# whaiproject/BetaZero

Measured on AMD Instinct MI355X. Metric: selfplay_games_per_s, higher is better.
Workload: dtype bf16

## Files before the change

betazero_amd/csrc/bz_mcts.hip:

```cpp
#include <new>

#include <time.h>

#include "bz_common.h"
#include "bz_math.h"
#include "bz_rules.h"
#include "bz_fpu.h"
#include "bz_solver.h"
#include "bz_early_stop.h"
#include "bz_options.h"
#include "bz_pace.h"
#include "bz_gumbel_interior.h"
#include "bz_surprise.h"
#include "bz_value.h"
#include "bz_ownership.h"
#include "bz_resign.h"

using namespace bz;

namespace {

struct __attribute__((aligned(16))) Node { u64 own, opp, legal; u32 edge0, info; };
struct __attribute__((aligned(16))) Edge { u32 w0; float W; float P; u32 w3; };
static_assert(sizeof(Node) == 32 && sizeof(Edge) == 16, "layout");
// ... 2231 lines not shown
    const int tm = E.g_to_move[g];
    uint8_t* st = R.streak + i * 2 + (tm == 1 ? 0 : 1);
    int s;
    const bool fire = resign_step(q, R.threshold, R.consecutive, (int)*st, &s);
    *st = (uint8_t)s;
    if (!fire) return;
    if (R.side[i] == 0) { R.side[i] = (int8_t)tm; R.move[i] = E.g_moves[g]; R.q[i] = q; }
    if (out) return;
    const int nex = E.g_nex[g] < E.t_max ? E.g_nex[g] : E.t_max, w = -tm;
    const size_t rowbase = i * E.t_max;
    for (int t = 0; t < nex; ++t) E.ex_z[rowbase + t] = (int8_t)(w * E.ex_mover[rowbase + t]);
    E.ex_len[i] = nex;
    E.ex_winner[i] = (int8_t)w;
    atomicAdd(&E.flags[FLAG_FINISHED], 1u);
    E.g_state[g] = kStateResigned;
}
template <class G>
__global__ void __launch_bounds__(256) k_resign_finish(EngineDev E, int restart) {
    const int g = blockIdx.x * blockDim.x + threadIdx.x;
    if (g >= E.B || E.g_state[g] != kStateResigned) return;
    const int round = E.g_round[g];
    if (restart && round + 1 < E.rounds) { dev_start_game<G>(E, g, round + 1); return; }
    E.g_state[g] = 1;
}

__global__ void __launch_bounds__(256) k_pack_own(EngineDev E, OwnDev O, u64* fown, u64* fopp, int64_t cap) {
    dev_pack_walk(E, cap, [=](int i, size_t s, size_t d) {
        u64 a, b;
        ownership_row(O.fin_x[i], O.fin_o[i], (int)E.ex_mover[s], &a, &b);
        fown[d] = a; fopp[d] = b;
    });
}

struct __attribute__((aligned(64))) StoreHdr { u64 own, opp, epoch; u32 n_nodes, n_edges, ready, pad[7]; };
static_assert(sizeof(StoreHdr) == 64, "layout");
struct StoreDev {
    int S, D, n_idx, base;
    u32* n_used;
    u32* idx;
    StoreHdr* hdr;
    u32* mark;
    Node* nodes; Edge* edges; float* node_v; u64* tt;
};
constexpr int kCntSeededEvals = 11, kCntSeededSearches = 12, kCntStoreSaves = 13;
constexpr int kCntReplaySeeds = 14, kCntReplaySims = 15;

__device__ __forceinline__ u32 store_home(const StoreDev& St, u64 own, u64 opp) { return (u32)(hash_pos(own, opp) >> 20) & (u32)(St.n_idx - 1); }
__device__ __forceinline__ int store_find(const StoreDev& St, u64 own, u64 opp, u64 epoch, u32* at) {
    u32 p = store_home(St, own, opp);
    for (int k = 0; k < St.n_idx; ++k, p = (p + 1u) & (u32)(St.n_idx - 1)) {
        const u32 w = St.idx[p];
        if (w == 0u || w > (u32)St.S) { *at = p; return -1; }
        const StoreHdr& h = St.hdr[w - 1u];
        if (h.own == own && h.opp == opp && h.epoch == epoch) { *at = p; return (int)(w - 1u); }
    }
    *at = ~0u;
    return -1;
}
__device__ __forceinline__ bool store_depth_ok(const EngineDev& E, const StoreDev& St, int g) {
    const int d = E.g_moves[g] - St.base;
    return E.g_state[g] == 0 && d >= 0 && d < St.D;
}
__device__ __forceinline__ u32 tt_gen_before(u32 gen) { return gen == 1u ? kTtGenMax - 1u : gen - 1u; }

__device__ __forceinline__ bool tt_replay_from_prev(const EngineDev& E, int g, u32 i, u32 gen, u32 prev_nodes) {
    const Node nd = E.nodes[(size_t)g * E.ncap + i];
    if (nd.info & kTerm) return false;
#ifdef BZ_EXP_TT_WEAK_HASH
    const u64 h = hash_pos(nd.own, nd.opp) & 1u;
#else
    const u64 h = hash_pos(nd.own, nd.opp);
#endif
    const u32 tag = (u32)(h >> 32), gen_prev = tt_gen_before(gen);
    const u64* bucket = E.tt + ((size_t)g * (size_t)E.tt_buckets + (size_t)(h & (u64)(E.tt_buckets - 1))) * 16;
    u32 hit = ~0u;
    for (int s = 0; s < 16; ++s) {
        const u64 e = bucket[s];
        const u32 meta = (u32)(e >> 32), egen = meta >> kChildBits;
        const bool cur = egen == gen && (meta & kChildMask) < i, prv = prev_nodes != 0u && egen == gen_prev;
        if ((cur || prv) && (u32)e == tag) {
            const u32 key = ((prv ? 1u : 0u) << 20) | ((u32)s << 16) | (meta & kChildMask);
            hit = key < hit ? key : hit;
        }
    }
    if (hit == ~0u || (hit >> 20) == 0u) return false;
    const u32 x = hit & kChildMask;
    if (x == 0u || x >= prev_nodes) return false;
    const Node xn = E.nodes_alt[(size_t)g * E.ncap + x];
    return xn.own == nd.own && xn.opp == nd.opp && !(xn.info & kTerm) && (xn.info & 0xFFu) != 0u;
}

__global__ void __launch_bounds__(256) k_store_save(EngineDev E, StoreDev St, u32 gen, u64 epoch, const u32* budget) {
    __shared__ int claim[256];
    __shared__ u32 part[256];
    const int t = threadIdx.x;
    if ((int)blockIdx.x < E.B) {
        const int g = blockIdx.x;
        const GameHot& hot = E.hot[g];
        if (E.g_state[g] != 0 || hot.tt_gen != gen || hot.last_gen != gen || hot.prev_nodes == 0u || St.mark[g] != tt_gen_before(gen)) return;
        const u32 n = hot.n_nodes < (u32)E.ncap ? hot.n_nodes : (u32)E.ncap;
        u32 mine = 0;
        for (u32 i = 1u + (u32)t; i < n; i += 256u) mine += tt_replay_from_prev(E, g, i, gen, hot.prev_nodes) ? 1u : 0u;
        part[t] = mine;
        __syncthreads();
        for (int o = 128; o > 0; o >>= 1) { if (t < o) part[t] += part[t + o]; __syncthreads(); }
        if (t == 0 && part[0]) atomicAdd(reinterpret_cast<unsigned long long*>(E.counters) + kCntSeededEvals, (unsigned long long)part[0]);
        return;
    }
    const size_t ttn = (size_t)E.tt_buckets * 16;
    for (int g0 = 0; g0 < E.B; g0 += 256) {
        const int g = g0 + t;
        int c = -1;
        if (g < E.B && store_depth_ok(E, St, g) && E.hot[g].last_gen == gen && E.hot[g].tt_gen == gen && E.hot[g].n_nodes > 1u &&
            E.hot[g].n_nodes <= (u32)E.ncap && E.hot[g].n_edges <= (u32)E.ecap && !(budget && budget[g] < (u32)E.sims)) {
            const Node r = E.nodes[(size_t)g * E.ncap];
            u32 at;
            if (store_find(St, r.own, r.opp, epoch, &at) < 0) c = -2;
        }
        claim[t] = c;
        __syncthreads();
        if (t == 0) {
            for (int j = 0; j < 256; ++j) {
                if (claim[j] != -2) continue;
                claim[j] = -1;
                const u32 used = *St.n_used;
                if (used >= (u32)St.S) continue;
                const int gj = g0 + j;
                const Node r = E.nodes[(size_t)gj * E.ncap];
                u32 at;
                if (store_find(St, r.own, r.opp, epoch, &at) >= 0 || at == ~0u) continue;
                StoreHdr h{};
                h.own = r.own; h.opp = r.opp; h.epoch = epoch; h.n_nodes = E.hot[gj].n_nodes; h.n_edges = E.hot[gj].n_edges; h.ready = 0u;
                St.hdr[used] = h;
                St.idx[at] = used + 1u;
                *St.n_used = used + 1u;
                __threadfence();
                claim[j] = (int)used;
            }
        }
        __syncthreads();
        for (int j = 0; j < 256; ++j) {
            const int en = claim[j];
            if (en < 0) continue;
            const int gj = g0 + j;
            const u32 nn = St.hdr[en].n_nodes, ne = St.hdr[en].n_edges;
            const uint4* sn = reinterpret_cast<const uint4*>(E.nodes + (size_t)gj * E.ncap);
            uint4* dn = reinterpret_cast<uint4*>(St.nodes + (size_t)en * E.ncap);
            for (u32 k = t; k < nn * 2u; k += 256u) dn[k] = sn[k];
            const uint4* se = reinterpret_cast<const uint4*>(E.edges + (size_t)gj * E.ecap);
            uint4* de = reinterpret_cast<uint4*>(St.edges + (size_t)en * E.ecap);
            for (u32 k = t; k < ne; k += 256u) de[k] = se[k];
            const float* sv = E.node_v + (size_t)gj * E.ncap;
            float* dv = St.node_v + (size_t)en * E.ncap;
            for (u32 k = t; k < nn; k += 256u) dv[k] = sv[k];
            const u64* st = E.tt + (size_t)gj * ttn;
            u64* dt = St.tt + (size_t)en * ttn;
            for (size_t k = t; k < ttn; k += 256) {
                const u64 e = st[k];
                dt[k] = ((u32)(e >> 32) >> kChildBits) == gen ? e : 0ULL;
            }
        }
        __syncthreads();
        if (t == 0)
            for (int j = 0; j < 256; ++j)
                if (claim[j] >= 0) {
                    St.hdr[claim[j]].ready = 1u;
                    atomicAdd(reinterpret_cast<unsigned long long*>(E.counters) + kCntStoreSaves, 1ULL);
                }
        __syncthreads();
    }
}

__global__ void __launch_bounds__(256) k_store_seed(EngineDev E, StoreDev St, u32 gen, u64 epoch) {
    __shared__ int found;
    const int g = blockIdx.x, t = threadIdx.x;
    if (t == 0) {
        int en = -1;
        if (store_depth_ok(E, St, g)) {
            u32 at;
            en = store_find(St, E.g_own[g], E.g_opp[g], epoch, &at);
            if (en >= 0 && (St.hdr[en].ready == 0u || St.hdr[en].n_nodes > (u32)E.ncap || St.hdr[en].n_edges > (u32)E.ecap)) en = -1;
        }
        found = en;
    }
    __syncthreads();
    const int en = found;
    if (en < 0) return;
    const u32 nn = St.hdr[en].n_nodes, ne = St.hdr[en].n_edges;
    const uint4* sn = reinterpret_cast<const uint4*>(St.nodes + (size_t)en * E.ncap);
    uint4* dn = reinterpret_cast<uint4*>(E.nodes + (size_t)g * E.ncap);
    for (u32 k = t; k < nn * 2u; k += 256u) dn[k] = sn[k];
    const uint4* se = reinterpret_cast<const uint4*>(St.edges + (size_t)en * E.ecap);
    uint4* de = reinterpret_cast<uint4*>(E.edges + (size_t)g * E.ecap);
    for (u32 k = t; k < ne; k += 256u) de[k] = se[k];
    const float* sv = St.node_v + (size_t)en * E.ncap;
    float* dv = E.node_v + (size_t)g * E.ncap;
    for (u32 k = t; k < nn; k += 256u) dv[k] = sv[k];
    const size_t ttn = (size_t)E.tt_buckets * 16;
    const u64* st = St.tt + (size_t)en * ttn;
    u64* dt = E.tt + (size_t)g * ttn;
    for (size_t k = t; k < ttn; k += 256) {
        const u64 e = st[k];
// ... 643 lines not shown
}

static bool root_prep(const bz_engine* e) { return e->dev.dir_eps > 0.0f || e->gumbel.m > 0; }
static bool search_is_fused(const bz_engine* e) {
    const int ek = e->cfg.eval_kind;
    return (ek == BZ_EVAL_UNIFORM || ek == BZ_EVAL_HASH) && !e->dev.reuse && !root_prep(e) && engine_mode(e) == 0u;
}

constexpr int kPaceAutoSlots = 1024;
static int32_t paced_search(bz_engine* e, void* stream) {
    const int from_prev = e->seed_src;
    const bool plain = engine_mode(e) == 0u && !(e->dev.dir_eps > 0.0f) && !e->dev.reuse && !e->sym_on && e->dev.ecache == 2 &&
                       net_eval(e->cfg.eval_kind) && e->cfg.game != BZ_GAME_TTT && e->dev.compact;
    if (!plain || e->replay_seed == 0 || (e->replay_seed == 2 && e->dev.B <= kPaceAutoSlots)) return BZ_OK;
    const size_t lds = (size_t)e->dev.ncap * 8;
    const u32* mark = e->store.S > 0 ? e->store.mark : nullptr;
#define BZ_SEED(G) hipLaunchKernelGGL(k_replay_seed<G>, dim3(e->dev.B), dim3(G::GW), lds, (hipStream_t)stream, e->dev, e->search_seq, from_prev, mark)
    switch (e->cfg.game) {
    case BZ_GAME_REVERSI6: BZ_SEED(Reversi6); break;
    case BZ_GAME_REVERSI4: BZ_SEED(Reversi4); break;
    default: BZ_SEED(Reversi); break;
    }
#undef BZ_SEED
    BZ_LAUNCH_CHECK("k_replay_seed");
    e->paced = 1;
    return BZ_OK;
}

static int32_t store_save(bz_engine* e, void* stream) {
    if (e->store.S == 0) return BZ_OK;
    hipLaunchKernelGGL(k_store_save, dim3(e->dev.B + 1), dim3(256), 0, (hipStream_t)stream, e->dev, e->store, e->search_seq, e->eval_epoch,
                       cap_budgets(e));
    BZ_LAUNCH_CHECK("k_store_save");
    return BZ_OK;
}

BZ_EXPORT int32_t bz_engine_search(bz_engine* e, void* stream) {
    BZ_REQUIRE(e, "null engine");
    int ek = e->cfg.eval_kind;
    const bool noise = root_prep(e);
    if (search_is_fused(e)) {
        ProfScope ps(BZ_PROF_SEARCH_FUSED, stream);
        if (e->cfg.game == BZ_GAME_TTT && e->cfg.sims <= kTttFusedMaxSims && e->ttt_gw > 0) {
            const dim3 grid = grid_groups(e->dev.B, e->ttt_gw);
#define BZ_TTT_FUSED(GWN)                                                                                              \
    do {                                                                                                                \
        if (ek == BZ_EVAL_UNIFORM) hipLaunchKernelGGL((k_search_fused_ttt<GWN, true>), grid, dim3(256), 0, (hipStream_t)stream, e->dev); \
        else hipLaunchKernelGGL((k_search_fused_ttt<GWN, false>), grid, dim3(256), 0, (hipStream_t)stream, e->dev);     \
    } while (0)
            switch (e->ttt_gw) {
            case 1: BZ_TTT_FUSED(1); break;
            case 2: BZ_TTT_FUSED(2); break;
            case 8: BZ_TTT_FUSED(8); break;
            default: BZ_TTT_FUSED(4); break;
            }
#undef BZ_TTT_FUSED
            BZ_LAUNCH_CHECK("k_search_fused_ttt");
            return BZ_OK;
        }
        BZ_DISPATCH_G(e, k_search_fused, stream, e->dev, ek);
        return BZ_OK;
    }
    BZ_REQUIRE(ek != BZ_EVAL_EXTERNAL, "bz_engine_search: BZ_EVAL_EXTERNAL callers drive the step API");
    int32_t rc;
    if ((rc = bz_engine_root_begin(e, stream)) != BZ_OK) return rc;
    if ((rc = paced_search(e, stream)) != BZ_OK) return rc;
// ... 880 lines not shown
```

betazero_amd/csrc/bz_net.hip:

```cpp
#include <limits.h>
#include <math.h>
#include <stdlib.h>
#include <new>
#include <atomic>
#include <vector>

#include "bz_common.h"
#include "bz_math.h"
#include "bz_sym.h"
#include "bz_tower.h"

using namespace bz;

using namespace bz_tower;

struct bz_net {
    int C, NB, VH, max_batch;
    float *stem_w, *stem_b;
    float *conv_w, *conv_b;
    __bf16* conv_wf;
    __bf16 *stem_wf, *head_wf;
    __bf16 *conv_wf16, *stem_wf16;
    uint8_t *conv_wf8, *head_wf8;
    float *dq8, *head_dq8, *ones;
// ... 40 lines not shown
            int src[8];
#pragma unroll
            for (int j = 0; j < 8; ++j) {
                int cell = c0 + j, yy = (cell >> 3) + dy, xx = (cell & 7) + dx;
                src[j] = (yy < 0 || yy > 7 || xx < 0 || xx > 7) ? -1 : (yy * 8 + xx) * C;
            }
            const float* wt = w + (size_t)t * C * C + co;
            for (int ci = 0; ci < C; ++ci) {
                float wv = wt[(size_t)ci * C];
#pragma unroll
                for (int j = 0; j < 8; ++j)
                    if (src[j] >= 0) acc[j] = __builtin_fmaf(xs[src[j] + ci], wv, acc[j]);
            }
        }
#pragma unroll
        for (int j = 0; j < 8; ++j) {
            size_t o = ((size_t)pos * 64 + c0 + j) * C + co;
            float v = acc[j];
            if (skip) v = v + skip[o];
            out[o] = relu_f32(v);
        }
    }
}

typedef Tw<64, 2> TwS64;
typedef Tw<128, 1> TwS128;
typedef Tw<256, 1> TwS256;
typedef Tw<128, 4, true> TwM16;
typedef Tw<128, 4, true, 1> TwEdge;
constexpr int kSmallBatch = 256;
constexpr int kAdaptT1 = 256;
enum { kShapeLatency = 0, kShapeMiddle = 1, kShapeThroughput = 2, kShapes = 4 };

struct TowerArgs {
    const u64 *own, *opp;
    const u32* n_dev;
    int n, n_layers, VH;
    int lo, hi;
    u32* tally;
    const uint4* wf;
    const uint4 *wf16, *stem_wf16;
    const float* bias;
    const uint4* stem_wf;
    const float* stem_b;
    const uint4* head_wf;
    const uint4 *wf8, *head_wf8;
    const float *dq8, *head_dq8, *ones;
    const float *pol_b, *val_b;
    const float *polfc_wT, *polfc_b;
    const float *v1_wT, *v1_b, *v2_w, *v2_b;
    float *logits, *value;
};

__device__ __forceinline__ unsigned nbhd(u64 b, int cell) {
    const int s = cell - 9;
    const u64 w = s >= 0 ? b >> s : b << -s;
    unsigned n = (unsigned)w & 0x00070707u;
    const int x = cell & 7;
    if (x == 0) n &= ~0x00010101u;
    if (x == 7) n &= ~0x00040404u;
    return n;
}
template <int KC>
__device__ __forceinline__ bf16x8 stem_frag(unsigned n_own, unsigned n_opp, int h) {
    unsigned wd[4];
#pragma unroll
// ... 201 lines not shown
    BZ_STAMP(t3);
    tacc[0] += t1 - t0; tacc[1] += t2 - t1; tacc[2] += t3 - t2;
}

#define BZ_NET_SYM 0
#include "bz_net_tower_fp8_body.h"
#undef BZ_NET_SYM
#define BZ_NET_SYM 1
#include "bz_net_tower_fp8_body.h"
#undef BZ_NET_SYM
}

__global__ void __launch_bounds__(256) k_sym_mean(const float* __restrict__ part, int n, float* __restrict__ logits,
                                                  float* __restrict__ value) {
    const int64_t nl = (int64_t)n * 65, total = nl + n;
    for (int64_t i = blockIdx.x * (int64_t)256 + threadIdx.x; i < total; i += (int64_t)gridDim.x * 256) {
        const bool isv = i >= nl;
        const float* src = isv ? part + 8 * nl + (i - nl) : part + i;
        const int64_t stride = isv ? n : nl;
        float acc = src[0] + src[stride];
#pragma unroll
        for (int s = 2; s < 8; ++s) acc = acc + src[s * stride];
        acc = acc * 0.125f;
        if (isv) value[i - nl] = acc; else logits[i] = acc;
    }
}

struct Carver {
    int64_t off = 0;
    int64_t take(int64_t bytes) { int64_t o = off; off += (bytes + 255) & ~int64_t(255); return o; }
};
struct NetOffsets {
    int64_t stem_w, stem_b, conv_w, conv_b, conv_wf, stem_wf, head_wf, conv_wf16, stem_wf16, conv_wf8, head_wf8, dq8, head_dq8, ones, pol_w, pol_b, polfc_wT, polfc_b, val_w, val_b, v1_wT, v1_b, v2_w,
        v2_b, act_a, act_b, tally, total;
};
NetOffsets net_carve(int C, int NB, int VH, int mb) {
    NetOffsets o{};
    Carver k;
    int64_t L = 2 * NB, mbp = (mb + 7) & ~7;
    o.stem_w = k.take(18LL * C * 4); o.stem_b = k.take(C * 4LL);
    o.conv_w = k.take(L * 9 * C * C * 4); o.conv_b = k.take(L * C * 4);
    const bool mfma = C == 64 || C == 128 || C == 256;
    const int64_t KC = C / 16, MT = C / 32;
    o.conv_wf = k.take(mfma ? (L * 9 + 2) * KC * MT * 1024 : 0);
    o.stem_wf = k.take(mfma ? 2 * MT * 1024 : 0); o.head_wf = k.take(mfma ? KC * 1024 : 0);
    o.conv_wf16 = k.take(C == kTC ? (L * 9 + 2) * (C / 32) * MT * 2 * 1024 : 0);
    o.stem_wf16 = k.take(C == kTC ? MT * 2 * 1024 : 0);
    o.conv_wf8 = k.take(C == kTC ? (L * 9 + 1) * 2LL * 4 * 2 * 64 * 16 : 0); o.head_wf8 = k.take(2 * 2 * 64 * 16);
    o.dq8 = k.take((L + 1) * 128 * 4); o.head_dq8 = k.take(16); o.ones = k.take(128 * 4);
    o.pol_w = k.take(2LL * C * 4); o.pol_b = k.take(8); o.polfc_wT = k.take(128 * 65 * 4); o.polfc_b = k.take(65 * 4);
    o.val_w = k.take(C * 4LL); o.val_b = k.take(4); o.v1_wT = k.take(64LL * VH * 4); o.v1_b = k.take(VH * 4LL);
    o.v2_w = k.take(VH * 4LL); o.v2_b = k.take(4);
    o.act_a = k.take(mbp * 64 * C * 4); o.act_b = k.take(mbp * 64 * C * 4);
    o.tally = k.take(kShapes * 4);
    o.total = k.off;
    return o;
}
bool shape_ok(int C, int NB, int VH, int mb) {
    return (C == 32 || C == 64 || C == 128 || C == 256) && NB >= 0 && NB <= 64 && VH >= 1 && VH <= 64 && mb >= 1;
}
uint16_t f2bf(float f) {
    u32 u;
    __builtin_memcpy(&u, &f, 4);
    if ((u & 0x7F800000u) == 0x7F800000u) return (uint16_t)((u >> 16) | ((u & 0x7FFFFFu) ? 0x40u : 0u));
    return (uint16_t)((u + 0x7FFFu + ((u >> 16) & 1u)) >> 16);
}
uint8_t f2e4m3(float f) {
    uint8_t sign = f < 0.0f ? 0x80 : 0;
    float a = fabsf(f);
    if (!(a == a)) return 0x7F;
    if (a > 448.0f) a = 448.0f;
    if (a == 0.0f) return sign;
    int ex;
    (void)frexpf(a, &ex);
    int e = ex - 1 < -6 ? -6 : ex - 1;
    float q = nearbyintf(a / ldexpf(1.0f, e - 3)) * ldexpf(1.0f, e - 3);
    if (q > 448.0f) q = 448.0f;
    if (q == 0.0f) return sign;
    (void)frexpf(q, &ex);
    int e2 = ex - 1;
    if (e2 < -6) return sign | (uint8_t)nearbyintf(q * 512.0f);
    int mant = (int)nearbyintf((q / ldexpf(1.0f, e2) - 1.0f) * 8.0f);
    return sign | (uint8_t)(((e2 + 7) << 3) | mant);
}
float pow2_scale(float maxabs) {
// ... 66 lines not shown
                        size_t f = (((((size_t)l * 9 + t) * (C / 32) + kq) * MT + wt) * 2 + a) * 64 + (g * 16 + c);
                        w16[f * 8 + j] = f2bf(v);
                    }
                }
        q += (size_t)C * C * 9;
        for (int i = 0; i < C; ++i) F(o.conv_b)[(size_t)l * C + i] = q[i];
        q += C;
    }
    if (C == kTC) {
        uint8_t* w8 = reinterpret_cast<uint8_t*>(img.data() + o.conv_wf8);
        for (int l = 0; l < L; ++l) {
            const float* wl = F(o.conv_w) + (size_t)l * 9 * C * C;
            for (int co = 0; co < C; ++co) {
                float mx = 0.0f;
                for (int t = 0; t < 9; ++t)
                    for (int ci = 0; ci < C; ++ci) mx = fmaxf(mx, fabsf(wl[((size_t)t * C + ci) * C + co]));
                const float sc = pow2_scale(mx);
                F(o.dq8)[(size_t)l * C + co] = 1.0f / (sc * 16.0f);
                for (int t = 0; t < 9; ++t)
                    for (int ci = 0; ci < C; ++ci) {
                        int ks = ci >> 6, hh = (ci >> 5) & 1, j = ci & 31, half = j >> 4, mt = co >> 5, rr = co & 31;
                        size_t f = ((((((size_t)l * 9 + t) * 2 + ks) * 4 + mt) * 2 + half) * 64 + (hh * 32 + rr)) * 16 + (j & 15);
                        w8[f] = f2e4m3(wl[((size_t)t * C + ci) * C + co] * sc);
                    }
            }
        }
        for (int i = 0; i < 128; ++i) F(o.ones)[i] = 1.0f;
    }
    for (int i = 0; i < 2 * C; ++i) F(o.pol_w)[i] = q[i];
    q += 2 * C;
    F(o.pol_b)[0] = q[0]; F(o.pol_b)[1] = q[1]; q += 2;
    for (int a = 0; a < 65; ++a)
        for (int i = 0; i < 128; ++i) F(o.polfc_wT)[i * 65 + a] = q[a * 128 + i];
    q += 65 * 128;
    for (int a = 0; a < 65; ++a) F(o.polfc_b)[a] = q[a];
    q += 65;
    for (int i = 0; i < C; ++i) F(o.val_w)[i] = q[i];
    q += C;
    F(o.val_b)[0] = q[0]; q += 1;
    for (int hh = 0; hh < VH; ++hh)
        for (int i = 0; i < 64; ++i) F(o.v1_wT)[i * VH + hh] = q[hh * 64 + i];
    q += (size_t)VH * 64;
    for (int i = 0; i < VH; ++i) F(o.v1_b)[i] = q[i];
    q += VH;
    for (int i = 0; i < VH; ++i) F(o.v2_w)[i] = q[i];
    q += VH;
    F(o.v2_b)[0] = q[0];
    if (mfma) {
        uint16_t* hf = reinterpret_cast<uint16_t*>(img.data() + o.head_wf);
        for (int kc = 0; kc < KC; ++kc)
            for (int ln = 0; ln < 64; ++ln)
                for (int j = 0; j < 8; ++j) {
                    int row = ln & 31, k = 16 * kc + 8 * (ln >> 5) + j;
                    float v = row < 2 ? F(o.pol_w)[row * C + k] : (row == 2 ? F(o.val_w)[k] : 0.0f);
                    hf[((size_t)kc * 64 + ln) * 8 + j] = f2bf(v);
                }
    }
    if (C == kTC) {
        uint8_t* h8 = reinterpret_cast<uint8_t*>(img.data() + o.head_wf8);
        float hs[3];
        for (int row = 0; row < 3; ++row) {
            float mx = 0.0f;
            for (int k = 0; k < C; ++k) mx = fmaxf(mx, fabsf(row < 2 ? F(o.pol_w)[row * C + k] : F(o.val_w)[k]));
            hs[row] = pow2_scale(mx);
            F(o.head_dq8)[row] = 1.0f / (hs[row] * 16.0f);
        }
        for (int ks = 0; ks < 2; ++ks)
            for (int ln = 0; ln < 64; ++ln)
                for (int j = 0; j < 32; ++j) {
                    int row = ln & 31, k = 64 * ks + 32 * (ln >> 5) + j;
                    float v = row < 2 ? F(o.pol_w)[row * C + k] * hs[row] : (row == 2 ? F(o.val_w)[k] * hs[2] : 0.0f);
                    h8[((size_t)(ks * 2 + (j >> 4)) * 64 + ln) * 16 + (j & 15)] = f2e4m3(v);
                }
    }
// ... 305 lines not shown
```

betazero_amd/csrc/bz_net_tower_bf16_body.h:

```cpp

template <class G>
__global__ void __launch_bounds__(256, 1)
#if BZ_NET_SYM
k_sym_bf16(TowerArgs T, bz_sym::Args Y) {
#elif BZ_NET_EDGE
k_edge_bf16(TowerArgs T) {
#else
k_tower_bf16(TowerArgs T) {
#endif
    constexpr int C = G::C, P = G::P, PW = G::PW, MW = G::MW;
    extern __shared__ __attribute__((aligned(16))) char smem[];
    const int tid = threadIdx.x, lane = tid & 63;
    const int w = __builtin_amdgcn_readfirstlane(tid >> 6);
    const int pos0 = blockIdx.x * P;
    const int cnt = T.n_dev ? (int)*T.n_dev : T.n;
    if ((unsigned)cnt - (unsigned)T.lo > (unsigned)T.hi - (unsigned)T.lo) return;
    T.n = cnt < T.n ? cnt : T.n;
    if (pos0 >= T.n) return;
    if (T.tally && blockIdx.x == 0 && tid == 0) atomicAdd(T.tally, 1u);
    [[maybe_unused]] unsigned long long tacc[4] = {0, 0, 0, 0}, tk0 = 0, tk1 = 0, tr0 = 0, tr1 = 0;
    BZ_STAMP(tk0);
#ifdef BZ_EXP_STAMPS
    tr0 = __builtin_amdgcn_s_memrealtime();
#endif
    char* bufX = smem;
    char* bufM = smem + G::BUF;
    const int r = lane & 31, h = lane >> 5;

    constexpr int ZC = G::CELL / 16;
    for (int i = tid; i < 2 * P * 9 * ZC; i += 256) {
        int k = i % ZC, j = (i / ZC) % 9, pb = i / (9 * ZC);
        *reinterpret_cast<uint4*>(smem + pb * G::TILE + j * G::ROWC * G::CELL + k * 16) = make_uint4(0, 0, 0, 0);
    }
    const int wt0 = G::wt0(w), wp0 = G::pos0(w);
    const uint4* ap = G::M16 ? T.wf16 + (size_t)wt0 * 2 * 64 : T.wf + (size_t)wt0 * 64;
    typename WSetsOf<G>::type WS;
    if constexpr (G::M16) {
#pragma unroll
        for (int kq = 0; kq < G::KQ; ++kq)
#pragma unroll
            for (int a = 0; a < 2; ++a) WS.s[0][kq][a] = __builtin_bit_cast(bf16x8, ap[(kq * G::MT * 2 + a) * 64 + (unsigned)lane]);
        ap += G::KQ * G::MT * 2 * 64;
    } else {
#pragma unroll
        for (int d = 0; d + 1 < G::DEPTH; ++d) {
#pragma unroll
            for (int kc = 0; kc < G::KS; ++kc)
#pragma unroll
                for (int mt = 0; mt < MW; ++mt) WS.s[d][kc][mt] = __builtin_bit_cast(bf16x8, ap[(kc * G::MT + mt) * 64 + (unsigned)lane]);
            ap += G::KS * G::MT * 64;
        }
    }

    if constexpr (G::EDGE) {
        namespace tmap = bz_tile_map;
        f32x16 acc[MW][G::NU];
        Bias<G> bias;
        const int c = lane & 15, g = lane >> 4;
        load_bias16<G>(bias, T.stem_b, wt0, g);
        bf16x8 sa[2];
#pragma unroll
        for (int a = 0; a < 2; ++a) sa[a] = __builtin_bit_cast(bf16x8, T.stem_wf16[(wt0 * 2 + a) * 64 + lane]);
        const int lp[5] = {tmap::lane_p(tmap::kRow, c), 2 + tmap::lane_p(tmap::kRow, c), tmap::lane_p(tmap::kCol, c),
                           tmap::lane_p(tmap::kMix, c), tmap::lane_p(tmap::kIn, c)};
        u64 own[5], opp[5];
#pragma unroll
        for (int i = 0; i < 5; ++i) {
            int pos = pos0 + wp0 + lp[i];
            pos = pos < T.n ? pos : T.n - 1;
            own[i] = T.own[pos]; opp[i] = T.opp[pos];
        }
#pragma unroll
        for (int u = 0; u < G::NU; ++u) {
            acc[0][u] = (f32x16)(0.0f);
#pragma unroll
            for (int b = 0; b < 2; ++b) {
                const int t = 2 * u + b, i = t < 4 ? (t & 1) : 1 + tmap::pattern(t);
                const int cell = 8 * tmap::pair_y(t, c) + tmap::pair_x(t, c);
                const bf16x8 f = stem_frag16(nbhd(own[i], cell), nbhd(opp[i], cell), g);
                if (b) { mfma16_quarter<1>(acc[0][u], sa[0], f); mfma16_quarter<3>(acc[0][u], sa[1], f); }
                else { mfma16_quarter<0>(acc[0][u], sa[0], f); mfma16_quarter<2>(acc[0][u], sa[1], f); }
            }
        }
        epilogue_edge<G>(acc, bufX + wp0 * G::TILE, false, bias, wt0, lane);
    } else if constexpr (G::M16) {
        f32x16 acc[MW][G::NU];
        Bias<G> bias;
        const int c = lane & 15, g = lane >> 4;
        load_bias16<G>(bias, T.stem_b, wt0, g);
        bf16x8 sa[2];
#pragma unroll
        for (int a = 0; a < 2; ++a) sa[a] = __builtin_bit_cast(bf16x8, T.stem_wf16[(wt0 * 2 + a) * 64 + lane]);
        u64 own[2], opp[2];
#pragma unroll
        for (int b = 0; b < 2; ++b) {
            int pos = pos0 + wp0 + 2 * b + (c >> 3);
            pos = pos < T.n ? pos : T.n - 1;
            own[b] = T.own[pos]; opp[b] = T.opp[pos];
#if BZ_NET_SYM
            {
                const u32 s = bz_sym::of(Y, own[b], opp[b]);
                own[b] = bz_sym::board(own[b], Y.size, s); opp[b] = bz_sym::board(opp[b], Y.size, s);
            }
// ... 30 lines not shown
#if BZ_NET_SYM
            {
                const u32 s = bz_sym::of(Y, own[i], opp[i]);
                own[i] = bz_sym::board(own[i], Y.size, s); opp[i] = bz_sym::board(opp[i], Y.size, s);
            }
#endif
        }
#pragma unroll
        for (int u = 0; u < G::NU; ++u) {
            const int i = G::ROWT ? 0 : u >> 1;
            const int cell = G::unit_cell(u, r);
            const unsigned n_own = nbhd(own[i], cell), n_opp = nbhd(opp[i], cell);
            bf16x8 sf[2] = {stem_frag<0>(n_own, n_opp, h), stem_frag<1>(n_own, n_opp, h)};
#pragma unroll
            for (int mt = 0; mt < MW; ++mt) {
                acc[mt][u] = (f32x16)(0.0f);
#pragma unroll
                for (int kc = 0; kc < 2; ++kc)
                    acc[mt][u] = __builtin_amdgcn_mfma_f32_32x32x16_bf16(sa[kc][mt], sf[kc], acc[mt][u], 0, 0, 0);
            }
        }
        epilogue<G>(acc, bufX + wp0 * G::TILE, false, bias, wt0, r, h);
    }
    __syncthreads();

#pragma unroll 1
    for (int blk = 0; blk < T.n_layers / 2; ++blk) {
        conv_layer<0, G>(bufX, bufM, false, T.bias + (size_t)(2 * blk) * C, WS, ap, w, r, h, tacc);
        conv_layer<G::NCH % G::DEPTH, G>(bufM, bufX, true, T.bias + (size_t)(2 * blk + 1) * C, WS, ap, w, r, h, tacc);
    }
    BZ_STAMP(tk1);

    float* S = reinterpret_cast<float*>(bufM + w * 1024);
    const float pb0 = T.pol_b[0], pb1 = T.pol_b[1], vb = T.val_b[0];
    bf16x8 hw[G::KC];
#pragma unroll
    for (int kc = 0; kc < G::KC; ++kc) hw[kc] = __builtin_bit_cast(bf16x8, T.head_wf[kc * 64 + lane]);
    for (int p = w; p < P && pos0 + p < T.n; p += 4) {
        const int pos = pos0 + p;
#if BZ_NET_SYM
        const int dst = bz_sym::tau_inv(Y.size, bz_sym::of(Y, T.own[pos], T.opp[pos]), lane);
#else
        const int dst = lane;
#endif
#pragma unroll
        for (int nt = 0; nt < 2; ++nt) {
            f32x16 acc = (f32x16)(0.0f);
            const int cell = 32 * nt + r;
#pragma unroll
            for (int kc = 0; kc < G::KC; ++kc) {
                bf16x8 b = *reinterpret_cast<const bf16x8*>(bufX + p * G::TILE + G::cell_off(p, cell, 2 * kc + h));
                acc = __builtin_amdgcn_mfma_f32_32x32x16_bf16(hw[kc], b, acc, 0, 0, 0);
            }
            if (h == 0) {
                float a0 = acc[0] + pb0, a1 = acc[1] + pb1, a2 = acc[2] + vb;
                S[cell] = relu_f32(a0);
                S[64 + cell] = relu_f32(a1);
                S[128 + cell] = relu_f32(a2);
            }
        }
        __builtin_amdgcn_s_waitcnt(0xC07F);
        float acc = T.polfc_b[lane], part = 0.0f;
#pragma unroll 8
        for (int i = 0; i < 128; i += 4) {
            f32x4 s4 = *reinterpret_cast<const f32x4*>(S + i);
#pragma unroll
            for (int j = 0; j < 4; ++j) acc = __builtin_fmaf(s4[j], T.polfc_wT[(i + j) * 65 + lane], acc);
        }
        part = S[lane] * T.polfc_wT[lane * 65 + 64] + S[lane + 64] * T.polfc_wT[(lane + 64) * 65 + 64];
        part = wave_sum(part);
        T.logits[(size_t)pos * 65 + dst] = acc;
        if (lane == 0) T.logits[(size_t)pos * 65 + 64] = part + T.polfc_b[64];
        float vh = 0.0f;
        if (lane < T.VH) {
            float a = T.v1_b[lane];
#pragma unroll 32
            for (int i = 0; i < 64; ++i) a = __builtin_fmaf(S[128 + i], T.v1_wT[i * T.VH + lane], a);
            vh = relu_f32(a) * T.v2_w[lane];
        }
        vh = wave_sum(vh);
        if (lane == 0) T.value[pos] = tanhf_spec(vh + T.v2_b[0]);
        __builtin_amdgcn_s_waitcnt(0xC07F);
    }
#ifdef BZ_EXP_STAMPS
    unsigned long long tk2; BZ_STAMP(tk2);
    tr1 = __builtin_amdgcn_s_memrealtime();
    if (tid == 0 && blockIdx.x < 4096) {
        unsigned long long* d = g_dbg + blockIdx.x * 8;
        d[0] = tacc[0]; d[1] = tacc[1]; d[2] = tacc[2]; d[3] = tk1 - tk0; d[4] = tk2 - tk0; d[5] = tr1 - tr0; d[6] = tk0; d[7] = tr0;
    }
#endif
}
```

betazero_amd/csrc/bz_tower.h:

```cpp
#pragma once
#include "bz_common.h"
#include "bz_tile_map.h"

typedef __attribute__((ext_vector_type(8))) __bf16 bf16x8;
typedef __attribute__((ext_vector_type(4))) __bf16 bf16x4;
typedef __attribute__((ext_vector_type(2))) __bf16 bf16x2;
typedef __attribute__((ext_vector_type(4))) short s16x4;
typedef __attribute__((ext_vector_type(2))) short s16x2;
typedef __attribute__((ext_vector_type(2))) float f32x2;
typedef __attribute__((ext_vector_type(4))) float f32x4;
typedef __attribute__((ext_vector_type(16))) float f32x16;

namespace bz_tower {
using namespace bz;
constexpr int kTC = 128;

template <int C_, int P_ = 512 / C_, bool M16_ = false, int MAP_ = 0> struct Tw {
    static_assert(C_ == 64 || C_ == 128 || C_ == 256, "the MFMA tower is built for 64, 128 or 256 channels");
    static constexpr int C = C_;
    static constexpr bool EDGE = MAP_ == 1;
    static_assert(MAP_ == 0 || (MAP_ == 1 && M16_ && C_ == 128 && P_ == 4), "the edge-aware tiling serves Tw<128, 4, true> only");
    static constexpr bool M16 = M16_;
    static constexpr int KQ = C / 32;
    static constexpr int KC = C / 16;
// ... 327 lines not shown
                                           int lane) {
    const int c = lane & 15, g = lane >> 4, x = c & 7, pl = c >> 3;
    int home2[2] = {pl * G::TILE + G::cell_at(0, x) + 8 * (g & 1), pl * G::TILE + G::cell_at(1, x) + 8 * (g & 1)};
    asm volatile("" : "+v"(home2[0]), "+v"(home2[1]));
#pragma unroll
    for (int a = 0; a < 2; ++a) {
        const int slot = G::pos16(4 * wt + 2 * a + (g >> 1), x);
        const f32x4 bq = bias.q[0][a];
#pragma unroll
        for (int b = 0; b < 2; ++b)
#pragma unroll
            for (int par = 0; par < 2; ++par)
#pragma unroll
                for (int u = par; u < G::NU; u += 2) {
                    const int off = home2[par] + slot + b * 2 * G::TILE + (u & ~1) * G::ROWC * G::CELL;
                    const int q = 2 * a + b;
                    f32x4 v = {acc[0][u][4 * q], acc[0][u][4 * q + 1], acc[0][u][4 * q + 2], acc[0][u][4 * q + 3]};
                    v = v + bq;
                    if (second) {
                        bf16x4 sk = *reinterpret_cast<const bf16x4*>(out + off);
                        v = v + __builtin_convertvector(sk, f32x4);
                    }
                    v = relu_f32x4(v);
                    f32x2 vlo = {v[0], v[1]}, vhi = {v[2], v[3]};
                    s16x2 lo = __builtin_bit_cast(s16x2, __builtin_convertvector(vlo, bf16x2));
                    s16x2 hi = __builtin_bit_cast(s16x2, __builtin_convertvector(vhi, bf16x2));
                    *reinterpret_cast<uint2*>(out + off) = make_uint2(__builtin_bit_cast(unsigned, lo), __builtin_bit_cast(unsigned, hi));
                }
    }
}

namespace tmap = bz_tile_map;
struct EdgeOff { int o[tmap::kPatterns][8]; };
template <class G>
__device__ __forceinline__ void edge_offsets(EdgeOff& E, int c, int sub, int rot0, int extra) {
#pragma unroll
    for (int pat = 0; pat < tmap::kPatterns; ++pat)
#pragma unroll
        for (int u = 0; u < 8; ++u)
            E.o[pat][u] = tmap::lane_cells(pat, c) * G::CELL + (tmap::lane_slot(pat, c, sub, (u + rot0) & 7) << 4) + extra;
}
template <class G, int TAP>
__device__ __forceinline__ void load_b_edge(bf16x8 (&b)[G::NU], const char* in, const EdgeOff& E, int kq, int hf) {
#pragma unroll
    for (int j = 0; j < G::NU; ++j) {
        const int t = 2 * j + hf;
        if (!tmap::skip(TAP, t))
            b[j] = *reinterpret_cast<const bf16x8*>(in + E.o[tmap::pattern(t)][tmap::slot_rot(t, TAP, 4 * kq)] +
                                                    (tmap::tile_cells(t) + tmap::tap_cells(TAP)) * G::CELL);
    }
}
template <class G, int TAP, int HF>
__device__ __forceinline__ void mfma_edge(f32x16 (&acc)[G::MW][G::NU], const bf16x8 (&a)[2], const bf16x8 (&b)[G::NU]) {
#pragma unroll
    for (int j = 0; j < G::NU; ++j)
        if (!tmap::skip(TAP, 2 * j + HF)) {
            mfma16_quarter<HF>(acc[0][j], a[0], b[j]);
            mfma16_quarter<2 + HF>(acc[0][j], a[1], b[j]);
        }
}
template <int S, int TAP, class G>
__device__ __forceinline__ void tap_step_edge(f32x16 (&acc)[G::MW][G::NU], WSets16<G>& WS, const uint4*& ap, const char* in,
                                              const EdgeOff& E, int lane, bf16x8 (&B)[2][G::NU]) {
    constexpr bool last = TAP == 8;
    constexpr int TAP_N = last ? TAP : TAP + 1;
    bf16x8 (&use)[G::KQ][2] = WS.s[S];
// ... 142 lines not shown
```

Baseline: 253.6.

## Parallelize store copy per game, prefetch edge-tower inputs, and restructure the fused policy/value head

The store save kernel, which used to copy each claimed game's tree serially inside a single block, now only claims slots. A new per-game kernel copies nodes, edges, values and the transposition table in parallel across blocks. The edge-aware bf16 tower now loads stem weights, biases and board bitboards before the early-exit checks to hide their latency, and uses a new head path with one position per wave. That head reads packed lane-major FC weights held in registers and interleaves their loads with the MFMAs. This adds a kernel launch, uses more registers, and performs some loads for blocks that may then exit.

```diff
diff --git a/betazero_amd/csrc/bz_mcts.hip b/betazero_amd/csrc/bz_mcts.hip
--- a/betazero_amd/csrc/bz_mcts.hip
+++ b/betazero_amd/csrc/bz_mcts.hip
@@ -2287,7 +2287,7 @@
     });
 }
 
-struct __attribute__((aligned(64))) StoreHdr { u64 own, opp, epoch; u32 n_nodes, n_edges, ready, pad[7]; };
+struct __attribute__((aligned(64))) StoreHdr { u64 own, opp, epoch; u32 n_nodes, n_edges, ready, slot, pad[6]; };
 static_assert(sizeof(StoreHdr) == 64, "layout");
 struct StoreDev {
     int S, D, n_idx, base;
@@ -2315,6 +2315,10 @@
 __device__ __forceinline__ bool store_depth_ok(const EngineDev& E, const StoreDev& St, int g) {
     const int d = E.g_moves[g] - St.base;
     return E.g_state[g] == 0 && d >= 0 && d < St.D;
+}
+__device__ __forceinline__ bool store_wants(const EngineDev& E, const StoreDev& St, int g, u32 gen, const u32* budget) {
+    return store_depth_ok(E, St, g) && E.hot[g].last_gen == gen && E.hot[g].tt_gen == gen && E.hot[g].n_nodes > 1u &&
+           E.hot[g].n_nodes <= (u32)E.ncap && E.hot[g].n_edges <= (u32)E.ecap && !(budget && budget[g] < (u32)E.sims);
 }
 __device__ __forceinline__ u32 tt_gen_before(u32 gen) { return gen == 1u ? kTtGenMax - 1u : gen - 1u; }
 
@@ -2362,12 +2366,10 @@
         if (t == 0 && part[0]) atomicAdd(reinterpret_cast<unsigned long long*>(E.counters) + kCntSeededEvals, (unsigned long long)part[0]);
         return;
     }
-    const size_t ttn = (size_t)E.tt_buckets * 16;
     for (int g0 = 0; g0 < E.B; g0 += 256) {
         const int g = g0 + t;
         int c = -1;
-        if (g < E.B && store_depth_ok(E, St, g) && E.hot[g].last_gen == gen && E.hot[g].tt_gen == gen && E.hot[g].n_nodes > 1u &&
-            E.hot[g].n_nodes <= (u32)E.ncap && E.hot[g].n_edges <= (u32)E.ecap && !(budget && budget[g] < (u32)E.sims)) {
+        if (g < E.B && store_wants(E, St, g, gen, budget)) {
             const Node r = E.nodes[(size_t)g * E.ncap];
             u32 at;
             if (store_find(St, r.own, r.opp, epoch, &at) < 0) c = -2;
@@ -2386,43 +2388,55 @@
                 if (store_find(St, r.own, r.opp, epoch, &at) >= 0 || at == ~0u) continue;
                 StoreHdr h{};
                 h.own = r.own; h.opp = r.opp; h.epoch = epoch; h.n_nodes = E.hot[gj].n_nodes; h.n_edges = E.hot[gj].n_edges; h.ready = 0u;
+                h.slot = (u32)gj + 1u;
                 St.hdr[used] = h;
                 St.idx[at] = used + 1u;
                 *St.n_used = used + 1u;
                 __threadfence();
-                claim[j] = (int)used;
             }
         }
         __syncthreads();
-        for (int j = 0; j < 256; ++j) {
-            const int en = claim[j];
-            if (en < 0) continue;
-            const int gj = g0 + j;
-            const u32 nn = St.hdr[en].n_nodes, ne = St.hdr[en].n_edges;
-            const uint4* sn = reinterpret_cast<const uint4*>(E.nodes + (size_t)gj * E.ncap);
-            uint4* dn = reinterpret_cast<uint4*>(St.nodes + (size_t)en * E.ncap);
-            for (u32 k = t; k < nn * 2u; k += 256u) dn[k] = sn[k];
-            const uint4* se = reinterpret_cast<const uint4*>(E.edges + (size_t)gj * E.ecap);
-            uint4* de = reinterpret_cast<uint4*>(St.edges + (size_t)en * E.ecap);
-            for (u32 k = t; k < ne; k += 256u) de[k] = se[k];
-            const float* sv = E.node_v + (size_t)gj * E.ncap;
-            float* dv = St.node_v + (size_t)en * E.ncap;
-            for (u32 k = t; k < nn; k += 256u) dv[k] = sv[k];
-            const u64* st = E.tt + (size_t)gj * ttn;
-            u64* dt = St.tt + (size_t)en * ttn;
-            for (size_t k = t; k < ttn; k += 256) {
-                const u64 e = st[k];
-                dt[k] = ((u32)(e >> 32) >> kChildBits) == gen ? e : 0ULL;
-            }
-        }
-        __syncthreads();
-        if (t == 0)
-            for (int j = 0; j < 256; ++j)
-                if (claim[j] >= 0) {
-                    St.hdr[claim[j]].ready = 1u;
-                    atomicAdd(reinterpret_cast<unsigned long long*>(E.counters) + kCntStoreSaves, 1ULL);
-                }
-        __syncthreads();
+    }
+}
+
+__global__ void __launch_bounds__(256) k_store_copy(EngineDev E, StoreDev St, u32 gen, u64 epoch, const u32* budget) {
+    __shared__ int found;
+    const int g = blockIdx.x, t = threadIdx.x;
+    if (t == 0) {
+        int en = -1;
+        if (store_wants(E, St, g, gen, budget)) {
+            const Node r = E.nodes[(size_t)g * E.ncap];
+            u32 at;
+            en = store_find(St, r.own, r.opp, epoch, &at);
+            if (en >= 0 && (St.hdr[en].ready != 0u || St.hdr[en].slot != (u32)g + 1u)) en = -1;
+        }
+        found = en;
+    }
+    __syncthreads();
+    const int en = found;
+    if (en < 0) return;
+    const size_t ttn = (size_t)E.tt_buckets * 16;
+    const u32 nn = St.hdr[en].n_nodes, ne = St.hdr[en].n_edges;
+    const uint4* sn = reinterpret_cast<const uint4*>(E.nodes + (size_t)g * E.ncap);
+    uint4* dn = reinterpret_cast<uint4*>(St.nodes + (size_t)en * E.ncap);
+    for (u32 k = t; k < nn * 2u; k += 256u) dn[k] = sn[k];
+    const uint4* se = reinterpret_cast<const uint4*>(E.edges + (size_t)g * E.ecap);
+    uint4* de = reinterpret_cast<uint4*>(St.edges + (size_t)en * E.ecap);
+    for (u32 k = t; k < ne; k += 256u) de[k] = se[k];
+    const float* sv = E.node_v + (size_t)g * E.ncap;
+    float* dv = St.node_v + (size_t)en * E.ncap;
+    for (u32 k = t; k < nn; k += 256u) dv[k] = sv[k];
+    const u64* st = E.tt + (size_t)g * ttn;
+    u64* dt = St.tt + (size_t)en * ttn;
+    for (size_t k = t; k < ttn; k += 256) {
+        const u64 e = st[k];
+        dt[k] = ((u32)(e >> 32) >> kChildBits) == gen ? e : 0ULL;
+    }
+    __threadfence();
+    __syncthreads();
+    if (t == 0) {
+        St.hdr[en].ready = 1u;
+        atomicAdd(reinterpret_cast<unsigned long long*>(E.counters) + kCntStoreSaves, 1ULL);
     }
 }
 
@@ -3132,6 +3146,9 @@
     hipLaunchKernelGGL(k_store_save, dim3(e->dev.B + 1), dim3(256), 0, (hipStream_t)stream, e->dev, e->store, e->search_seq, e->eval_epoch,
                        cap_budgets(e));
     BZ_LAUNCH_CHECK("k_store_save");
+    hipLaunchKernelGGL(k_store_copy, dim3(e->dev.B), dim3(256), 0, (hipStream_t)stream, e->dev, e->store, e->search_seq, e->eval_epoch,
+                       cap_budgets(e));
+    BZ_LAUNCH_CHECK("k_store_copy");
     return BZ_OK;
 }
 
diff --git a/betazero_amd/csrc/bz_net.hip b/betazero_amd/csrc/bz_net.hip
--- a/betazero_amd/csrc/bz_net.hip
+++ b/betazero_amd/csrc/bz_net.hip
@@ -96,6 +96,10 @@
 constexpr int kAdaptT1 = 256;
 enum { kShapeLatency = 0, kShapeMiddle = 1, kShapeThroughput = 2, kShapes = 4 };
 
+constexpr int kPkBase = 128 * 65;
+static_assert(kPkBase % 4 == 0, "the lane-major copy is read 16 bytes at a time");
+constexpr int kPkPol = 0, kPkV1 = kPkPol + 32 * 64 * 4, kPkPass = kPkV1 + 16 * 64 * 4, kPkFloats = kPkPass + 2 * 64;
+
 struct TowerArgs {
     const u64 *own, *opp;
     const u32* n_dev;
@@ -363,7 +367,7 @@
 };
 struct NetOffsets {
     int64_t stem_w, stem_b, conv_w, conv_b, conv_wf, stem_wf, head_wf, conv_wf16, stem_wf16, conv_wf8, head_wf8, dq8, head_dq8, ones, pol_w, pol_b, polfc_wT, polfc_b, val_w, val_b, v1_wT, v1_b, v2_w,
-        v2_b, act_a, act_b, tally, total;
+        v2_b, fc_pk, act_a, act_b, tally, total;
 };
 NetOffsets net_carve(int C, int NB, int VH, int mb) {
     NetOffsets o{};
@@ -379,9 +383,10 @@
     o.stem_wf16 = k.take(C == kTC ? MT * 2 * 1024 : 0);
     o.conv_wf8 = k.take(C == kTC ? (L * 9 + 1) * 2LL * 4 * 2 * 64 * 16 : 0); o.head_wf8 = k.take(2 * 2 * 64 * 16);
     o.dq8 = k.take((L + 1) * 128 * 4); o.head_dq8 = k.take(16); o.ones = k.take(128 * 4);
-    o.pol_w = k.take(2LL * C * 4); o.pol_b = k.take(8); o.polfc_wT = k.take(128 * 65 * 4); o.polfc_b = k.take(65 * 4);
+    o.pol_w = k.take(2LL * C * 4); o.pol_b = k.take(8); o.polfc_wT = k.take((kPkBase + kPkFloats) * 4LL); o.polfc_b = k.take(65 * 4);
     o.val_w = k.take(C * 4LL); o.val_b = k.take(4); o.v1_wT = k.take(64LL * VH * 4); o.v1_b = k.take(VH * 4LL);
     o.v2_w = k.take(VH * 4LL); o.v2_b = k.take(4);
+    o.fc_pk = o.polfc_wT + kPkBase * 4LL;
     o.act_a = k.take(mbp * 64 * C * 4); o.act_b = k.take(mbp * 64 * C * 4);
     o.tally = k.take(kShapes * 4);
     o.total = k.off;
@@ -514,6 +519,9 @@
     F(o.pol_b)[0] = q[0]; F(o.pol_b)[1] = q[1]; q += 2;
     for (int a = 0; a < 65; ++a)
         for (int i = 0; i < 128; ++i) F(o.polfc_wT)[i * 65 + a] = q[a * 128 + i];
+    for (int a = 0; a < 64; ++a)
+        for (int i = 0; i < 128; ++i) F(o.fc_pk)[kPkPol + ((i >> 2) * 64 + a) * 4 + (i & 3)] = q[a * 128 + i];
+    for (int a = 0; a < 128; ++a) F(o.fc_pk)[kPkPass + a] = q[64 * 128 + a];
     q += 65 * 128;
     for (int a = 0; a < 65; ++a) F(o.polfc_b)[a] = q[a];
     q += 65;
@@ -521,7 +529,10 @@
     q += C;
     F(o.val_b)[0] = q[0]; q += 1;
     for (int hh = 0; hh < VH; ++hh)
-        for (int i = 0; i < 64; ++i) F(o.v1_wT)[i * VH + hh] = q[hh * 64 + i];
+        for (int i = 0; i < 64; ++i) {
+            F(o.v1_wT)[i * VH + hh] = q[hh * 64 + i];
+            F(o.fc_pk)[kPkV1 + ((i >> 2) * 64 + hh) * 4 + (i & 3)] = q[hh * 64 + i];
+        }
     q += (size_t)VH * 64;
     for (int i = 0; i < VH; ++i) F(o.v1_b)[i] = q[i];
     q += VH;
diff --git a/betazero_amd/csrc/bz_net_tower_bf16_body.h b/betazero_amd/csrc/bz_net_tower_bf16_body.h
--- a/betazero_amd/csrc/bz_net_tower_bf16_body.h
+++ b/betazero_amd/csrc/bz_net_tower_bf16_body.h
@@ -14,6 +14,31 @@
     const int w = __builtin_amdgcn_readfirstlane(tid >> 6);
     const int pos0 = blockIdx.x * P;
     const int cnt = T.n_dev ? (int)*T.n_dev : T.n;
+    [[maybe_unused]] EdgeEarly<G> early;
+    typename WSetsOf<G>::type WS;
+    if constexpr (G::EDGE) {
+        namespace tmap = bz_tile_map;
+        const int ewt = G::wt0(w), c = lane & 15, g = lane >> 4;
+        const int lp[5] = {tmap::lane_p(tmap::kRow, c), 2 + tmap::lane_p(tmap::kRow, c), tmap::lane_p(tmap::kCol, c),
+                           tmap::lane_p(tmap::kMix, c), tmap::lane_p(tmap::kIn, c)};
+#pragma unroll
+        for (int i = 0; i < 5; ++i) {
+            early.pos[i] = pos0 + G::pos0(w) + lp[i];
+            const int pos = early.pos[i] < T.n ? early.pos[i] : T.n - 1;
+            early.own[i] = T.own[pos]; early.opp[i] = T.opp[pos];
+        }
+#pragma unroll
+        for (int a = 0; a < 2; ++a) {
+            early.sa[a] = __builtin_bit_cast(bf16x8, T.stem_wf16[(ewt * 2 + a) * 64 + lane]);
+            early.bq[a] = *reinterpret_cast<const f32x4*>(T.stem_b + 32 * ewt + 16 * a + 4 * g);
+        }
+#pragma unroll
+        for (int kq = 0; kq < G::KQ; ++kq)
+#pragma unroll
+            for (int a = 0; a < 2; ++a)
+                WS.s[0][kq][a] = __builtin_bit_cast(bf16x8, T.wf16[(size_t)ewt * 2 * 64 + (kq * G::MT * 2 + a) * 64 + (unsigned)lane]);
+        asm volatile("" ::: "memory");
+    }
     if ((unsigned)cnt - (unsigned)T.lo > (unsigned)T.hi - (unsigned)T.lo) return;
     T.n = cnt < T.n ? cnt : T.n;
     if (pos0 >= T.n) return;
@@ -34,8 +59,9 @@
     }
     const int wt0 = G::wt0(w), wp0 = G::pos0(w);
     const uint4* ap = G::M16 ? T.wf16 + (size_t)wt0 * 2 * 64 : T.wf + (size_t)wt0 * 64;
-    typename WSetsOf<G>::type WS;
-    if constexpr (G::M16) {
+    if constexpr (G::EDGE) {
+        ap += G::KQ * G::MT * 2 * 64;
+    } else if constexpr (G::M16) {
 #pragma unroll
         for (int kq = 0; kq < G::KQ; ++kq)
 #pragma unroll
@@ -57,18 +83,14 @@
         f32x16 acc[MW][G::NU];
         Bias<G> bias;
         const int c = lane & 15, g = lane >> 4;
-        load_bias16<G>(bias, T.stem_b, wt0, g);
-        bf16x8 sa[2];
-#pragma unroll
-        for (int a = 0; a < 2; ++a) sa[a] = __builtin_bit_cast(bf16x8, T.stem_wf16[(wt0 * 2 + a) * 64 + lane]);
-        const int lp[5] = {tmap::lane_p(tmap::kRow, c), 2 + tmap::lane_p(tmap::kRow, c), tmap::lane_p(tmap::kCol, c),
-                           tmap::lane_p(tmap::kMix, c), tmap::lane_p(tmap::kIn, c)};
+        bias.q[0][0] = early.bq[0]; bias.q[0][1] = early.bq[1];
+        bias.q[0][2] = bias.q[0][3] = (f32x4)(0.0f);
+        const bf16x8 (&sa)[2] = early.sa;
         u64 own[5], opp[5];
 #pragma unroll
         for (int i = 0; i < 5; ++i) {
-            int pos = pos0 + wp0 + lp[i];
-            pos = pos < T.n ? pos : T.n - 1;
-            own[i] = T.own[pos]; opp[i] = T.opp[pos];
+            own[i] = early.own[i]; opp[i] = early.opp[i];
+            if (early.pos[i] >= T.n) { own[i] = T.own[T.n - 1]; opp[i] = T.opp[T.n - 1]; }
         }
 #pragma unroll
         for (int u = 0; u < G::NU; ++u) {
@@ -165,6 +187,84 @@
     BZ_STAMP(tk1);
 
     float* S = reinterpret_cast<float*>(bufM + w * 1024);
+    if constexpr (G::EDGE) {
+        static_assert(P == 4, "one head position per wave");
+        const int p = w, pos = pos0 + p;
+        if (pos < T.n) {
+            int hl = lane;
+            asm volatile("" : "+v"(hl));
+            const int hr = hl & 31, hh = hl >> 5;
+            bf16x8 hw[G::KC];
+#pragma unroll
+            for (int kc = 0; kc < G::KC; ++kc) hw[kc] = __builtin_bit_cast(bf16x8, T.head_wf[kc * 64 + hl]);
+            const float pb0 = T.pol_b[0], pb1 = T.pol_b[1], vb = T.val_b[0];
+            const float* pk = T.polfc_wT + kPkBase;
+            f32x4 pw[32], vw[16];
+#pragma unroll
+            for (int q = 0; q < 16; ++q) pw[q] = *reinterpret_cast<const f32x4*>(pk + kPkPol + (q * 64 + hl) * 4);
+            const float pfb = T.polfc_b[hl], pfb64 = T.polfc_b[64];
+            const float pc0 = pk[kPkPass + hl], pc1 = pk[kPkPass + 64 + hl];
+            const bool vlane = hl < T.VH;
+            const float v1b = vlane ? T.v1_b[hl] : 0.0f, v2w = vlane ? T.v2_w[hl] : 0.0f, v2b = T.v2_b[0];
+            bf16x8 b[2][G::KC];
+#pragma unroll
+            for (int nt = 0; nt < 2; ++nt)
+#pragma unroll
+                for (int kc = 0; kc < G::KC; ++kc)
+                    b[nt][kc] = *reinterpret_cast<const bf16x8*>(bufX + p * G::TILE + G::cell_off(p, 32 * nt + hr, 2 * kc + hh));
+            __builtin_amdgcn_sched_barrier(0);
+            f32x16 hacc[2] = {(f32x16)(0.0f), (f32x16)(0.0f)};
+#pragma unroll
+            for (int kc = 0; kc < G::KC; ++kc)
+#pragma unroll
+                for (int nt = 0; nt < 2; ++nt) hacc[nt] = __builtin_amdgcn_mfma_f32_32x32x16_bf16(hw[kc], b[nt][kc], hacc[nt], 0, 0, 0);
+#pragma unroll
+            for (int q = 16; q < 32; ++q) pw[q] = *reinterpret_cast<const f32x4*>(pk + kPkPol + (q * 64 + hl) * 4);
+            __builtin_amdgcn_sched_barrier(0);
+            if (hh == 0) {
+#pragma unroll
+                for (int nt = 0; nt < 2; ++nt) {
+                    const int cell = 32 * nt + hr;
+                    float a0 = hacc[nt][0] + pb0, a1 = hacc[nt][1] + pb1, a2 = hacc[nt][2] + vb;
+                    S[cell] = relu_f32(a0);
+                    S[64 + cell] = relu_f32(a1);
+                    S[128 + cell] = relu_f32(a2);
+                }
+            }
+            __builtin_amdgcn_s_waitcnt(0xC07F);
+            float acc = pfb;
+#pragma unroll
+            for (int q = 0; q < 16; ++q) {
+                f32x4 s4 = *reinterpret_cast<const f32x4*>(S + 4 * q);
+#pragma unroll
+                for (int j = 0; j < 4; ++j) acc = __builtin_fmaf(s4[j], pw[q][j], acc);
+            }
+            __builtin_amdgcn_sched_barrier(0);
+#pragma unroll
+            for (int q = 0; q < 16; ++q) vw[q] = *reinterpret_cast<const f32x4*>(pk + kPkV1 + (q * 64 + hl) * 4);
+            __builtin_amdgcn_sched_barrier(0);
+#pragma unroll
+            for (int q = 16; q < 32; ++q) {
+                f32x4 s4 = *reinterpret_cast<const f32x4*>(S + 4 * q);
+#pragma unroll
+                for (int j = 0; j < 4; ++j) acc = __builtin_fmaf(s4[j], pw[q][j], acc);
+            }
+            float part = S[hl] * pc0 + S[hl + 64] * pc1;
+            part = wave_sum(part);
+            T.logits[(size_t)pos * 65 + hl] = acc;
+            if (hl == 0) T.logits[(size_t)pos * 65 + 64] = part + pfb64;
+            float a = v1b;
+#pragma unroll
+            for (int q = 0; q < 16; ++q) {
+                f32x4 s4 = *reinterpret_cast<const f32x4*>(S + 128 + 4 * q);
+#pragma unroll
+                for (int j = 0; j < 4; ++j) a = __builtin_fmaf(s4[j], vw[q][j], a);
+            }
+            float vh = vlane ? relu_f32(a) * v2w : 0.0f;
+            vh = wave_sum(vh);
+            if (hl == 0) T.value[pos] = tanhf_spec(vh + v2b);
+        }
+    } else {
     const float pb0 = T.pol_b[0], pb1 = T.pol_b[1], vb = T.val_b[0];
     bf16x8 hw[G::KC];
 #pragma unroll
@@ -215,6 +315,7 @@
         if (lane == 0) T.value[pos] = tanhf_spec(vh + T.v2_b[0]);
         __builtin_amdgcn_s_waitcnt(0xC07F);
     }
+    }
 #ifdef BZ_EXP_STAMPS
     unsigned long long tk2; BZ_STAMP(tk2);
     tr1 = __builtin_amdgcn_s_memrealtime();
diff --git a/betazero_amd/csrc/bz_tower.h b/betazero_amd/csrc/bz_tower.h
--- a/betazero_amd/csrc/bz_tower.h
+++ b/betazero_amd/csrc/bz_tower.h
@@ -383,6 +383,12 @@
 
 namespace tmap = bz_tile_map;
 struct EdgeOff { int o[tmap::kPatterns][8]; };
+template <class G> struct EdgeEarly {
+    bf16x8 sa[2];
+    f32x4 bq[2];
+    unsigned long long own[5], opp[5];
+    int pos[5];
+};
 template <class G>
 __device__ __forceinline__ void edge_offsets(EdgeOff& E, int c, int sub, int rot0, int extra) {
 #pragma unroll
```

Result: no change. 254.9, median of 6 (+0.5%).
